# PRBonn/OverlapNet

Measured on NVIDIA H100. Metric: scan-pairs/sec (overlap+yaw) at 64x900, higher is better.
Workload: dtype f16

## Files before the change

overlapnet_b200/csrc/hopper.cuh:

```cuda
#pragma once
#include <cuda_runtime.h>
#include <stdint.h>

namespace hopper {

__device__ __forceinline__ uint32_t smem_u32(const void* p) { return (uint32_t)__cvta_generic_to_shared(p); }

__device__ __forceinline__ void mbar_init(uint64_t* bar, uint32_t count) {
  asm volatile("mbarrier.init.shared::cta.b64 [%0], %1;" :: "r"(smem_u32(bar)), "r"(count) : "memory");
}
__device__ __forceinline__ void mbar_fence_init() { asm volatile("fence.mbarrier_init.release.cluster;" ::: "memory"); }
__device__ __forceinline__ void mbar_arrive(uint64_t* bar) {
  asm volatile("{\n\t.reg .b64 st;\n\tmbarrier.arrive.shared::cta.b64 st, [%0];\n\t}\n" :: "r"(smem_u32(bar)) : "memory");
}
__device__ __forceinline__ void mbar_arrive_expect_tx(uint64_t* bar, uint32_t bytes) {
  asm volatile("{\n\t.reg .b64 st;\n\tmbarrier.arrive.expect_tx.shared::cta.b64 st, [%0], %1;\n\t}\n"
               :: "r"(smem_u32(bar)), "r"(bytes) : "memory");
}
__device__ __forceinline__ bool mbar_try_wait(uint64_t* bar, uint32_t parity) {
  uint32_t ok;
  asm volatile("{\n\t.reg .pred p;\n\tmbarrier.try_wait.parity.shared::cta.b64 p, [%1], %2;\n\tselp.u32 %0, 1, 0, p;\n\t}\n"
               : "=r"(ok) : "r"(smem_u32(bar)), "r"(parity) : "memory");
  return ok != 0;
}
__device__ __forceinline__ bool mbar_wait(uint64_t* bar, uint32_t parity, long long max_cycles) {
  if (mbar_try_wait(bar, parity)) return true;
  const long long t0 = clock64();
  while (!mbar_try_wait(bar, parity))
    if (clock64() - t0 > max_cycles) return false;
  return true;
}
constexpr long long kMbarWaitCycles = 1ll << 28;

template <int D>
struct MbarRing {
  uint64_t full[D], empty[D];
  __device__ __forceinline__ void init(uint32_t consumer_arrivals) {
    for (int s = 0; s < D; ++s) { mbar_init(&full[s], 1); mbar_init(&empty[s], consumer_arrivals); }
  }
  static __device__ __forceinline__ uint32_t slot(uint32_t i) { return i % D; }
  static __device__ __forceinline__ uint32_t parity(uint32_t i) { return (i / D) & 1; }
  __device__ __forceinline__ bool acquire(uint32_t i, uint32_t bytes) {
    if (!mbar_wait(&empty[slot(i)], parity(i) ^ 1, kMbarWaitCycles)) return false;
    mbar_arrive_expect_tx(&full[slot(i)], bytes);
    return true;
  }
  __device__ __forceinline__ bool try_acquire(uint32_t i, uint32_t bytes) {
    if (!mbar_try_wait(&empty[slot(i)], parity(i) ^ 1)) return false;
    mbar_arrive_expect_tx(&full[slot(i)], bytes);
    return true;
  }
  __device__ __forceinline__ uint64_t* bar(uint32_t i) { return &full[slot(i)]; }
  __device__ __forceinline__ bool wait(uint32_t i) { return mbar_wait(&full[slot(i)], parity(i), kMbarWaitCycles); }
  __device__ __forceinline__ void release(uint32_t i) {
    __syncwarp();
    if ((threadIdx.x & 31) == 0) mbar_arrive(&empty[slot(i)]);
  }
};

#define PIPE_WAIT(ok, code) \
  if (!(ok)) { atomicExch(err, (code)); goto done; }
#define INFLIGHT_WAIT(ok, code) \
  if (!failed && !(ok)) { atomicExch(err, (code)); failed = true; }

__device__ __forceinline__ void named_bar_sync(int id, int count) {
  asm volatile("bar.sync %0, %1;" :: "r"(id), "r"(count) : "memory");
}

__device__ __forceinline__ void bulk_g2s(void* smem_dst, const void* gmem_src, uint32_t bytes, uint64_t* bar) {
  asm volatile("cp.async.bulk.shared::cluster.global.mbarrier::complete_tx::bytes [%0], [%1], %2, [%3];"
               :: "r"(smem_u32(smem_dst)), "l"(gmem_src), "r"(bytes), "r"(smem_u32(bar)) : "memory");
}

constexpr uint32_t kNoSwizzle = 0, kSwizzle128B = 1;
__device__ __forceinline__ uint64_t desc_kmajor(uint32_t smem_addr, uint32_t lbo, uint32_t sbo, uint32_t layout) {
  return (uint64_t)((smem_addr >> 4) & 0x3FFF) | ((uint64_t)((lbo >> 4) & 0x3FFF) << 16) |
         ((uint64_t)((sbo >> 4) & 0x3FFF) << 32) | ((uint64_t)layout << 62);
}
__device__ __forceinline__ void wgmma_fence() { asm volatile("wgmma.fence.sync.aligned;" ::: "memory"); }
__device__ __forceinline__ void wgmma_commit() { asm volatile("wgmma.commit_group.sync.aligned;" ::: "memory"); }
template <int N>
__device__ __forceinline__ void wgmma_wait() { asm volatile("wgmma.wait_group.sync.aligned %0;" :: "n"(N) : "memory"); }

__device__ __forceinline__ void wgmma_m64n64k16_rs(float (&d)[32], const uint32_t (&a)[4], uint64_t b_desc) {
  asm volatile(
      "{\n\t.reg .pred p;\n\tsetp.ne.b32 p, %37, 0;\n\t"
      "wgmma.mma_async.sync.aligned.m64n64k16.f32.f16.f16 {%0, %1, %2, %3, %4, %5, %6, %7, %8, %9, %10, %11, %12, %13, %14, %15, %16, %17, %18, %19, %20, %21, %22, %23, %24, %25, %26, %27, %28, %29, %30, %31}, {%32, %33, %34, %35}, %36, p, 1, 1, 0;\n\t}\n"
      : "+f"(d[0]), "+f"(d[1]), "+f"(d[2]), "+f"(d[3]), "+f"(d[4]), "+f"(d[5]), "+f"(d[6]), "+f"(d[7]), "+f"(d[8]), "+f"(d[9]), "+f"(d[10]), "+f"(d[11]), "+f"(d[12]), "+f"(d[13]), "+f"(d[14]), "+f"(d[15]), "+f"(d[16]), "+f"(d[17]), "+f"(d[18]), "+f"(d[19]), "+f"(d[20]), "+f"(d[21]), "+f"(d[22]), "+f"(d[23]), "+f"(d[24]), "+f"(d[25]), "+f"(d[26]), "+f"(d[27]), "+f"(d[28]), "+f"(d[29]), "+f"(d[30]), "+f"(d[31])
      : "r"(a[0]), "r"(a[1]), "r"(a[2]), "r"(a[3]), "l"(b_desc), "r"(1)
      : "memory");
}

__device__ __forceinline__ void wgmma_m64n128k16_ss(float (&d)[64], uint64_t a_desc, uint64_t b_desc) {
  asm volatile(
      "{\n\t.reg .pred p;\n\tsetp.ne.b32 p, %66, 0;\n\t"
      "wgmma.mma_async.sync.aligned.m64n128k16.f32.f16.f16 {%0, %1, %2, %3, %4, %5, %6, %7, %8, %9, %10, %11, %12, %13, %14, %15, %16, %17, %18, %19, %20, %21, %22, %23, %24, %25, %26, %27, %28, %29, %30, %31, %32, %33, %34, %35, %36, %37, %38, %39, %40, %41, %42, %43, %44, %45, %46, %47, %48, %49, %50, %51, %52, %53, %54, %55, %56, %57, %58, %59, %60, %61, %62, %63}, %64, %65, p, 1, 1, 0, 0;\n\t}\n"
      : "+f"(d[0]), "+f"(d[1]), "+f"(d[2]), "+f"(d[3]), "+f"(d[4]), "+f"(d[5]), "+f"(d[6]), "+f"(d[7]), "+f"(d[8]), "+f"(d[9]), "+f"(d[10]), "+f"(d[11]), "+f"(d[12]), "+f"(d[13]), "+f"(d[14]), "+f"(d[15]), "+f"(d[16]), "+f"(d[17]), "+f"(d[18]), "+f"(d[19]), "+f"(d[20]), "+f"(d[21]), "+f"(d[22]), "+f"(d[23]), "+f"(d[24]), "+f"(d[25]), "+f"(d[26]), "+f"(d[27]), "+f"(d[28]), "+f"(d[29]), "+f"(d[30]), "+f"(d[31]), "+f"(d[32]), "+f"(d[33]), "+f"(d[34]), "+f"(d[35]), "+f"(d[36]), "+f"(d[37]), "+f"(d[38]), "+f"(d[39]), "+f"(d[40]), "+f"(d[41]), "+f"(d[42]), "+f"(d[43]), "+f"(d[44]), "+f"(d[45]), "+f"(d[46]), "+f"(d[47]), "+f"(d[48]), "+f"(d[49]), "+f"(d[50]), "+f"(d[51]), "+f"(d[52]), "+f"(d[53]), "+f"(d[54]), "+f"(d[55]), "+f"(d[56]), "+f"(d[57]), "+f"(d[58]), "+f"(d[59]), "+f"(d[60]), "+f"(d[61]), "+f"(d[62]), "+f"(d[63])
      : "l"(a_desc), "l"(b_desc), "r"(1)
      : "memory");
}

}
```

overlapnet_b200/csrc/network_tc.cu:

```cuda
#include "common.cuh"
#include "hopper.cuh"

#include <cuda_fp16.h>
#include <stddef.h>
#include <stdlib.h>

namespace ovn {

using namespace hopper;

constexpr int WF = 360;
constexpr int CF = 128;
constexpr int S15 = 15;
constexpr int NB = 24;
constexpr int PAIR_ROWS = NB * NB;
constexpr int K4_PITCH = CF;

struct TcState {
  Buffer<__half> w1p;
  Buffer<__half> w2p;
  Buffer<__half> w3p;
  Buffer<float> b2eff;
  Buffer<__half> wres[kMaxLegLayers];
  Buffer<__half> actp[2];
  Buffer<float> leg_part;
  Buffer<__half> l16;
  Buffer<__half> r16;
  Buffer<__half> o1;
  Buffer<__half> x3;
  Buffer<float> partial;
  Buffer<__half> lc;
  Buffer<__half> rc;
  Buffer<float> corr_part;
  const float* pb_key = nullptr;
  int64_t pb_rows = 0;
  Buffer<__half> pb_l16;
  Buffer<__half> pb_lc;
  Buffer<float> mu;
  bool mu_set = false;
  Buffer<float> mu_o1;
  Buffer<float> mu_x3;
  Buffer<float> b2base;
  Buffer<float> b3eff;
  bool act_set = false;
  int64_t rows_pad = 0;
};

void TcStateDelete::operator()(TcState* t) const { delete t; }

__host__ __device__ __forceinline__ int k4_pos(int r, int c) {
  const int k = c & 31;
  return (((c >> 5) ^ (r & 1)) << 5) + ((k & 7) >> 1) * 8 + (k >> 3) * 2 + (k & 1);
}

__global__ void __launch_bounds__(256)
k_gather_rows_f16(const float* __restrict__ bank, const int32_t* __restrict__ idx, int n, const float* __restrict__ mu,
                  int row_shift, __half* __restrict__ out) {
  const int64_t per = (int64_t)WF * CF / 4;
  const int64_t i = (int64_t)blockIdx.x * blockDim.x + threadIdx.x;
  if (i >= (int64_t)n * per) return;
  const int p = (int)(i / per);
  const int64_t e = i % per;
  const int64_t row = idx ? idx[p] : p;
  const int r = (int)(e / (CF / 4)), c4 = (int)(e % (CF / 4));
  int64_t rs = r + row_shift;
  if (rs >= WF) rs -= WF;
  const float4 v = __ldg(reinterpret_cast<const float4*>(bank + (row * WF + rs) * CF) + c4);
  const float4 m = __ldg(reinterpret_cast<const float4*>(mu) + c4);
  __half2 a = __floats2half2_rn(v.x - m.x, v.y - m.y), b = __floats2half2_rn(v.z - m.z, v.w - m.w);
  __half* o = out + ((int64_t)p * WF + r) * K4_PITCH;
  *reinterpret_cast<uint32_t*>(o + k4_pos(r, 4 * c4)) = *reinterpret_cast<uint32_t*>(&a);
  *reinterpret_cast<uint32_t*>(o + k4_pos(r, 4 * c4 + 2)) = *reinterpret_cast<uint32_t*>(&b);
}

__global__ void __launch_bounds__(1024)
k_channel_mean(const float* __restrict__ bank, const int32_t* __restrict__ idx, int n, float* __restrict__ mu) {
  __shared__ float part[8][CF];
  const int c = threadIdx.x & (CF - 1), g = threadIdx.x >> 7;
  float acc = 0.f;
  for (int v = 0; v < n; ++v) {
    const float* vol = bank + (int64_t)(idx ? idx[v] : v) * WF * CF;
    for (int r = g; r < WF; r += 8) acc += __ldg(vol + (int64_t)r * CF + c);
  }
  part[g][c] = acc;
  __syncthreads();
  if (g == 0) {
    float t = 0.f;
    for (int k = 0; k < 8; ++k) t += part[k][c];
    mu[c] = __half2float(__float2half_rn(t / (float)((int64_t)n * WF)));
  }
}

constexpr int K4_STEPS = 60;

__host__ __device__ __forceinline__ size_t o1_chunk_offset(int64_t m, int di, int c8) {
  const int r = (int)(m & 127);
  return ((size_t)((m >> 7) * S15 + di) * 128 + r) * 64 + (size_t)((c8 ^ (r & 7)) * 8);
}

struct LegArgs {
  const __half* A; int64_t a_pitch;
  int runs_per_img, in_img_planes, in_run_planes;
  int kh, kw, c8in;
  const __half* Bp;
  const float* bias; int n_valid;
  int64_t M;
  __half* out_planes; int64_t out_pitch; int out_run_planes;
  float* out_f32;
  int n_split; float* part;
};

constexpr int C6_LROWS = 64, C6_RROWS = 128;
constexpr int C6_LT = 6, C6_RT = 3;
constexpr int C6_L_BYTES = 2 * 16 * C6_LROWS * 16;
constexpr int C6_R_BYTES = 2 * 16 * C6_RROWS * 16;
constexpr int C6_VOL_L_BYTES = C6_LT * C6_L_BYTES;
constexpr int C6_VOL_R_BYTES = C6_RT * C6_R_BYTES;

template <int TR, int NT>
__global__ void __launch_bounds__(256)
k_pack_corr(const float* __restrict__ bank, const int32_t* __restrict__ idx, int n, __half* __restrict__ out) {
  const int64_t i = (int64_t)blockIdx.x * blockDim.x + threadIdx.x;
  const int64_t per = 16 * NT * TR;
  if (i >= (int64_t)n * per) return;
  const int p = (int)(i / per);
  int r = (int)(i % per);
  const int vrow = r % (NT * TR); r /= NT * TR;
  const int pl = r;
  const int tile = vrow / TR, row = vrow % TR;
  float v[8];
  if (vrow < WF) {
    const int64_t src = (idx ? idx[p] : p);
    const float4 a = __ldg(reinterpret_cast<const float4*>(bank + (src * WF + vrow) * CF + pl * 8));
    const float4 b = __ldg(reinterpret_cast<const float4*>(bank + (src * WF + vrow) * CF + pl * 8 + 4));
    v[0] = a.x; v[1] = a.y; v[2] = a.z; v[3] = a.w; v[4] = b.x; v[5] = b.y; v[6] = b.z; v[7] = b.w;
  } else {
#pragma unroll
    for (int e = 0; e < 8; ++e) v[e] = 0.f;
  }
  __half hi[8], lo[8];
#pragma unroll
  for (int e = 0; e < 8; ++e) {
    hi[e] = __float2half_rn(v[e]);
    lo[e] = __float2half_rn(v[e] - __half2float(hi[e]));
  }
  __half* base = out + ((size_t)p * NT + tile) * (2 * 16 * TR * 8);
  *reinterpret_cast<uint4*>(base + ((size_t)pl * TR + row) * 8) = *reinterpret_cast<const uint4*>(hi);
  *reinterpret_cast<uint4*>(base + ((size_t)(16 + pl) * TR + row) * 8) = *reinterpret_cast<const uint4*>(lo);
}

constexpr int MMA_THREADS = 128;
constexpr int MMA_ROWS = 64;

__device__ __forceinline__ void mma16816(float (&d)[4], uint32_t a0, uint32_t a1, uint32_t a2, uint32_t a3,
                                         uint32_t b0, uint32_t b1) {
  asm volatile("mma.sync.aligned.m16n8k16.row.col.f32.f16.f16.f32 {%0,%1,%2,%3}, {%4,%5,%6,%7}, {%8,%9}, {%0,%1,%2,%3};"
               : "+f"(d[0]), "+f"(d[1]), "+f"(d[2]), "+f"(d[3])
               : "r"(a0), "r"(a1), "r"(a2), "r"(a3), "r"(b0), "r"(b1));
}

__device__ __forceinline__ uint32_t ld_h2(const __half* p) { return __ldg(reinterpret_cast<const unsigned int*>(p)); }

__device__ __forceinline__ uint32_t absdiff_h2(uint32_t a, uint32_t b) {
  const __half2 d = __hsub2(*reinterpret_cast<const __half2*>(&a), *reinterpret_cast<const __half2*>(&b));
  return *reinterpret_cast<const uint32_t*>(&d) & 0x7fff7fffu;
}

__device__ __forceinline__ uint32_t pack_h2(float a, float b) {
  const __half2 h = __floats2half2_rn(a, b);
  return *reinterpret_cast<const uint32_t*>(&h);
}

constexpr int K4_WG = 3;
constexpr int K4_THREADS = K4_WG * 128 + 32;
constexpr int K4_GROUP = 5;
constexpr int K4_NGROUPS = K4_STEPS / K4_GROUP;
static_assert(S15 % K4_GROUP == 0, "a W1 group within one 32-channel chunk");
constexpr int K4_RING = 4;
constexpr int K4_BSLICE = 4096;
constexpr uint32_t K4_VOL_BYTES = WF * K4_PITCH * 2;
constexpr uint32_t K4_RWIN_BYTES = S15 * K4_PITCH * 2;

struct K4Smem {
  __half L[WF * K4_PITCH];
  __half Rw[2][S15 * K4_PITCH];
  __half B[K4_RING][K4_GROUP * K4_BSLICE / 2];
  MbarRing<K4_RING> w1;
  MbarRing<1> left;
  MbarRing<2> right;
};
static_assert(sizeof(K4Smem) <= 232448, "k_delta_conv1_wgmma shared memory");
static_assert(offsetof(K4Smem, B) % 16 == 0 && offsetof(K4Smem, Rw) % 16 == 0, "bulk-copy alignment");

struct Share { int64_t begin, end; };
__device__ __forceinline__ Share work_share(int64_t n, uint32_t part, uint32_t parts) {
  return {n * part / parts, n * (part + 1) / parts};
}

__global__ void __launch_bounds__(K4_THREADS, 1)
k_delta_conv1_wgmma(const __half* __restrict__ L16, const int32_t* __restrict__ l_idx, const __half* __restrict__ R16,
                    int r_per_pair, const __half* __restrict__ W1p, const float* __restrict__ mu_o1,
                    __half* __restrict__ o1, int n_pairs, int* __restrict__ err) {
  extern __shared__ __align__(128) uint8_t smem_raw[];
  K4Smem& S = *reinterpret_cast<K4Smem*>(smem_raw);
  const int tid = threadIdx.x, warp = tid >> 5, lane = tid & 31;
  const Share share = work_share((int64_t)n_pairs * NB, blockIdx.x, gridDim.x);
  const int u_begin = (int)share.begin, u_end = (int)share.end;
  if (tid == 0) {
    S.w1.init(K4_WG * 4);
    S.left.init(K4_WG * 4);
    S.right.init(K4_WG * 4);
    mbar_fence_init();
  }
  __syncthreads();

  if (warp == K4_WG * 4) {
    if (lane == 0) {
      uint32_t pi = 0, gi = 0, ui = 0;
      for (int u = u_begin; u < u_end; ++u, ++ui) {
        const int p = u / NB, jb = u - p * NB;
        if (u == u_begin || jb == 0) {
          PIPE_WAIT(S.left.acquire(pi, K4_VOL_BYTES), kErrDeltaLeftProducer);
          bulk_g2s(S.L, L16 + (size_t)(l_idx ? l_idx[p] : p) * WF * K4_PITCH, K4_VOL_BYTES, S.left.bar(pi));
          ++pi;
        }
        PIPE_WAIT(S.right.acquire(ui, K4_RWIN_BYTES), kErrDeltaRightProducer);
        bulk_g2s(S.Rw[S.right.slot(ui)], R16 + (r_per_pair ? (size_t)p * WF * K4_PITCH : 0) + (size_t)jb * S15 * K4_PITCH,
                 K4_RWIN_BYTES, S.right.bar(ui));
        for (int grp = 0; grp < K4_NGROUPS; ++grp, ++gi) {
          PIPE_WAIT(S.w1.acquire(gi, K4_GROUP * K4_BSLICE), kErrDeltaW1Producer);
          bulk_g2s(S.B[S.w1.slot(gi)], W1p + (size_t)grp * K4_GROUP * (K4_BSLICE / 2), K4_GROUP * K4_BSLICE, S.w1.bar(gi));
        }
      }
    }
  } else {
    const int wg = warp >> 2, wi = warp & 3, g = lane >> 2, t = lane & 3;
    int rows[2][2];
#pragma unroll
    for (int tt = 0; tt < 2; ++tt) {
      const int r = (wg + 3 * tt) * 64 + wi * 16 + g;
      rows[tt][0] = r;
      rows[tt][1] = r + 8;
    }
    const uint32_t b_base = smem_u32(S.B[0]);
    uint32_t pi = 0, gi = 0, ui = 0;
    for (int u = u_begin; u < u_end; ++u, ++ui) {
      const int p = u / NB, jb = u - p * NB;
      if (u == u_begin || jb == 0) { PIPE_WAIT(S.left.wait(pi), kErrDeltaLeftConsumer); ++pi; }
      const uint32_t wb = S.right.slot(ui);
      PIPE_WAIT(S.right.wait(ui), kErrDeltaRightConsumer);
      float acc[2][32];
#pragma unroll
      for (int j = 0; j < 8; ++j) {
        const float m0 = __half2float(__float2half_rn(-__ldg(mu_o1 + j * 8 + 2 * t)));
        const float m1 = __half2float(__float2half_rn(-__ldg(mu_o1 + j * 8 + 2 * t + 1)));
#pragma unroll
        for (int tt = 0; tt < 2; ++tt) {
          acc[tt][4 * j + 0] = m0; acc[tt][4 * j + 1] = m1;
          acc[tt][4 * j + 2] = m0; acc[tt][4 * j + 3] = m1;
        }
      }
      uint32_t Lr[2][2][4];
#pragma unroll 1
      for (int grp = 0; grp < K4_NGROUPS; ++grp, ++gi) {
        const int cc = grp / 3, dj0 = (grp - 3 * cc) * K4_GROUP;
        if (dj0 == 0) {
#pragma unroll
          for (int tt = 0; tt < 2; ++tt)
#pragma unroll
            for (int h = 0; h < 2; ++h) {
              const int r = rows[tt][h] < WF ? rows[tt][h] : WF - 1;
              const uint4 v = *reinterpret_cast<const uint4*>(S.L + r * K4_PITCH + ((cc ^ (r & 1)) << 5) + 8 * t);
              Lr[tt][h][0] = v.x; Lr[tt][h][1] = v.y; Lr[tt][h][2] = v.z; Lr[tt][h][3] = v.w;
            }
        }
        const uint32_t s = S.w1.slot(gi);
        const uint64_t bdesc = desc_kmajor(b_base + s * (K4_GROUP * K4_BSLICE), 1024, 128, kNoSwizzle);
        const int par = (jb + dj0) & 1;
        const __half* rw = S.Rw[wb] + dj0 * K4_PITCH + 8 * t;
        const __half* rp[2] = {rw + ((cc ^ par) << 5), rw + ((cc ^ par ^ 1) << 5)};
        uint4 rv = *reinterpret_cast<const uint4*>(rp[0]);
        PIPE_WAIT(S.w1.wait(gi), kErrDeltaW1Consumer);
#pragma unroll
        for (int sl = 0; sl < K4_GROUP; ++sl) {
          uint32_t A[2][2][4];
#pragma unroll
          for (int tt = 0; tt < 2; ++tt) {
            A[tt][0][0] = absdiff_h2(Lr[tt][0][0], rv.x);
            A[tt][0][1] = absdiff_h2(Lr[tt][1][0], rv.x);
            A[tt][0][2] = absdiff_h2(Lr[tt][0][1], rv.y);
            A[tt][0][3] = absdiff_h2(Lr[tt][1][1], rv.y);
            A[tt][1][0] = absdiff_h2(Lr[tt][0][2], rv.z);
            A[tt][1][1] = absdiff_h2(Lr[tt][1][2], rv.z);
            A[tt][1][2] = absdiff_h2(Lr[tt][0][3], rv.w);
            A[tt][1][3] = absdiff_h2(Lr[tt][1][3], rv.w);
          }
          wgmma_fence();
#pragma unroll
          for (int kk = 0; kk < 2; ++kk)
#pragma unroll
            for (int tt = 0; tt < 2; ++tt)
              wgmma_m64n64k16_rs(acc[tt], A[tt][kk], bdesc + ((sl * K4_BSLICE + kk * 2048) >> 4));
          wgmma_commit();
          if (sl + 1 < K4_GROUP) rv = *reinterpret_cast<const uint4*>(rp[(sl + 1) & 1] + (sl + 1) * K4_PITCH);
          wgmma_wait<0>();
        }
        S.w1.release(gi);
      }
      S.right.release(ui);
      if (jb == NB - 1 || u == u_end - 1) S.left.release(pi - 1);
      const int64_t mrow = (int64_t)p * PAIR_ROWS + jb * NB;
#pragma unroll
      for (int tt = 0; tt < 2; ++tt)
#pragma unroll
        for (int h = 0; h < 2; ++h) {
          const int i = rows[tt][h];
          if (i >= WF) continue;
          const int ibk = i / S15, di = i - ibk * S15;
#pragma unroll
          for (int j = 0; j < 8; ++j)
            *reinterpret_cast<uint32_t*>(o1 + o1_chunk_offset(mrow + ibk, di, j) + 2 * t) =
                pack_h2(acc[tt][4 * j + 2 * h], acc[tt][4 * j + 2 * h + 1]);
        }
    }
  }
done:
  return;
}

constexpr int TC_WG = 2;
constexpr int TC_THREADS = TC_WG * 128 + 32;
constexpr int TC_ROWS = TC_WG * 128;
constexpr uint32_t C2_TILE = 128 * 64 * 2;
constexpr int C2_RING = 3;

struct C2Smem {
  __half A[C2_RING][TC_WG][C2_TILE / 2];
  __half B[C2_RING][2][C2_TILE / 2];
  MbarRing<C2_RING> ring;
};
constexpr size_t C2_SMEM = sizeof(C2Smem) + 1024;
static_assert(C2_SMEM <= 232448, "k_conv2_wgmma shared memory");
static_assert(offsetof(C2Smem, B) % 1024 == 0 && C2_TILE % 1024 == 0, "SWIZZLE_128B tiles on 1024-byte boundaries");

__global__ void __launch_bounds__(TC_THREADS, 1)
k_conv2_wgmma(const __half* __restrict__ o1, const __half* __restrict__ W2s, const float* __restrict__ bias2,
              const float* __restrict__ mu_x3, __half* __restrict__ x3, int64_t out_pitch, int64_t M, int fault,
              int* __restrict__ err) {
  if (fault) {
    if (threadIdx.x == 0 && blockIdx.x == 0) atomicExch(err, kErrInjectedFault);
    return;
  }
  extern __shared__ __align__(128) uint8_t smem_raw[];
  C2Smem& S = *reinterpret_cast<C2Smem*>(smem_raw + ((1024 - (smem_u32(smem_raw) & 1023)) & 1023));
  const int tid = threadIdx.x, warp = tid >> 5, lane = tid & 31;
  const Share tiles = work_share((M + TC_ROWS - 1) / TC_ROWS, blockIdx.x, gridDim.x);
  if (tid == 0) {
    S.ring.init(TC_WG * 4);
    mbar_fence_init();
  }
  __syncthreads();

  if (warp == TC_WG * 4) {
    if (lane == 0) {
      uint32_t gi = 0;
      for (int64_t tile = tiles.begin; tile < tiles.end; ++tile)
        for (int di = 0; di < S15; ++di, ++gi) {
          const uint32_t s = S.ring.slot(gi);
          PIPE_WAIT(S.ring.acquire(gi, 4 * C2_TILE), kErrConv2Producer);
          for (int h = 0; h < TC_WG; ++h)
            bulk_g2s(S.A[s][h], o1 + ((size_t)(tile * TC_WG + h) * S15 + di) * (C2_TILE / 2), C2_TILE, S.ring.bar(gi));
          bulk_g2s(S.B[s], W2s + (size_t)di * C2_TILE, 2 * C2_TILE, S.ring.bar(gi));
        }
    }
  } else {
    const int wg = warp >> 2, wi = warp & 3, g = lane >> 2, t = lane & 3;
    uint32_t gi = 0;
    bool failed = false;
    for (int64_t tile = tiles.begin; tile < tiles.end; ++tile) {
      float acc[2][64];
#pragma unroll
      for (int sub = 0; sub < 2; ++sub)
#pragma unroll
        for (int e = 0; e < 64; ++e) acc[sub][e] = 0.f;
#pragma unroll 1
      for (int di = 0; di < S15; ++di, ++gi) {
        const uint32_t s = S.ring.slot(gi);
        INFLIGHT_WAIT(S.ring.wait(gi), kErrConv2Consumer);
        const uint32_t a_base = smem_u32(S.A[s][wg]), b_base = smem_u32(S.B[s][0]);
        wgmma_fence();
#pragma unroll
        for (int kk = 0; kk < 4; ++kk)
#pragma unroll
          for (int part = 0; part < 2; ++part) {
            const uint64_t bd = desc_kmajor(b_base + part * C2_TILE + kk * 32, 16, 1024, kSwizzle128B);
#pragma unroll
            for (int sub = 0; sub < 2; ++sub)
              wgmma_m64n128k16_ss(acc[sub], desc_kmajor(a_base + sub * (C2_TILE / 2) + kk * 32, 16, 1024, kSwizzle128B), bd);
          }
        wgmma_commit();
        wgmma_wait<1>();
        if (di > 0) S.ring.release(gi - 1);
      }
      wgmma_wait<0>();
      if (failed) goto done;
      S.ring.release(gi - 1);
#pragma unroll
      for (int sub = 0; sub < 2; ++sub)
#pragma unroll
        for (int h = 0; h < 2; ++h) {
          const int64_t m = tile * TC_ROWS + wg * 128 + sub * 64 + wi * 16 + g + 8 * h;
          if (m >= M) continue;
#pragma unroll
          for (int j = 0; j < 16; ++j) {
            const int n = j * 8 + 2 * t;
            const float a = fmaxf(acc[sub][4 * j + 2 * h] + __ldg(bias2 + n), 0.f) - __ldg(mu_x3 + n);
            const float b = fmaxf(acc[sub][4 * j + 2 * h + 1] + __ldg(bias2 + n + 1), 0.f) - __ldg(mu_x3 + n + 1);
            *reinterpret_cast<uint32_t*>(x3 + ((size_t)j * out_pitch + m) * 8 + 2 * t) = pack_h2(a, b);
          }
        }
    }
  }
done:
  return;
}

constexpr int C3_AROWS = TC_ROWS + 2 * NB + 2;
constexpr uint32_t C3_PLANE = C3_AROWS * 16;
constexpr uint32_t C3_SLAB = 4 * 128 * 16;
constexpr int C3_GROUP = 2;
constexpr int C3_NSTAGES = 36 / C3_GROUP;
constexpr int C3_RING = 4;

struct C3Smem {
  __half A[2][16 * C3_PLANE / 2];
  __half B[C3_RING][C3_GROUP * C3_SLAB / 2];
  MbarRing<C3_RING> w3;
  MbarRing<2> x3;
};
static_assert(sizeof(C3Smem) <= 232448, "k_conv3_wgmma shared memory");
static_assert(offsetof(C3Smem, B) % 16 == 0 && C3_PLANE % 16 == 0, "bulk-copy alignment");

__global__ void __launch_bounds__(TC_THREADS, 1)
k_conv3_wgmma(const __half* __restrict__ X3, int64_t a_pitch, const __half* __restrict__ W3p, const float* __restrict__ bias,
              int64_t M, const float* __restrict__ wd, float* __restrict__ partial, int* __restrict__ err) {
  extern __shared__ __align__(128) uint8_t smem_raw[];
  C3Smem& S = *reinterpret_cast<C3Smem*>(smem_raw);
  const int tid = threadIdx.x, warp = tid >> 5, lane = tid & 31;
  const Share tiles = work_share(2 * ((M + TC_ROWS - 1) / TC_ROWS), blockIdx.x, gridDim.x);
  if (tid == 0) {
    S.w3.init(TC_WG * 4);
    S.x3.init(TC_WG * 4);
    mbar_fence_init();
  }
  __syncthreads();

  if (warp == TC_WG * 4) {
    if (lane == 0) {
      const uint32_t nt = (uint32_t)(tiles.end - tiles.begin);
      uint32_t ai = 0, gi = 0;
      for (uint32_t ti = 0; ti < nt; ++ti) {
        const int nh = (int)((tiles.begin + ti) & 1);
        for (int st = 0; st < C3_NSTAGES; ++st, ++gi) {
          while (ai < nt && ai <= ti + 1) {
            if (ai > ti) {
              if (!S.x3.try_acquire(ai, 16 * C3_PLANE)) break;
            } else {
              PIPE_WAIT(S.x3.acquire(ai, 16 * C3_PLANE), kErrConv3X3Producer);
            }
            const int64_t r0 = ((tiles.begin + ai) >> 1) * TC_ROWS;
            for (int pl = 0; pl < 16; ++pl)
              bulk_g2s(S.A[S.x3.slot(ai)] + pl * (C3_PLANE / 2), X3 + ((size_t)pl * a_pitch + r0) * 8, C3_PLANE, S.x3.bar(ai));
            ++ai;
          }
          PIPE_WAIT(S.w3.acquire(gi, C3_GROUP * C3_SLAB), kErrConv3W3Producer);
          bulk_g2s(S.B[S.w3.slot(gi)], W3p + ((size_t)nh * 36 + st * C3_GROUP) * (C3_SLAB / 2), C3_GROUP * C3_SLAB,
                   S.w3.bar(gi));
        }
      }
    }
  } else {
    const int wg = warp >> 2, wi = warp & 3, g = lane >> 2, t = lane & 3;
    const uint32_t b_base = smem_u32(S.B[0]);
    uint32_t gi = 0;
    bool failed = false;
    for (int64_t tile = tiles.begin; tile < tiles.end; ++tile) {
      const uint32_t ti = (uint32_t)(tile - tiles.begin);
      const int nh = (int)(tile & 1);
      const int64_t r0 = (tile >> 1) * TC_ROWS;
      PIPE_WAIT(S.x3.wait(ti), kErrConv3X3Consumer);
      const uint32_t a_rows = smem_u32(S.A[S.x3.slot(ti)]) + wg * 128 * 16;
      float acc[2][64];
#pragma unroll
      for (int sub = 0; sub < 2; ++sub)
#pragma unroll
        for (int e = 0; e < 64; ++e) acc[sub][e] = 0.f;
#pragma unroll 1
      for (int st = 0; st < C3_NSTAGES; ++st, ++gi) {
        const uint32_t s = S.w3.slot(gi);
        INFLIGHT_WAIT(S.w3.wait(gi), kErrConv3W3Consumer);
        wgmma_fence();
#pragma unroll
        for (int sl = 0; sl < C3_GROUP; ++sl) {
          const int slab = st * C3_GROUP + sl, tap = slab >> 2, c32 = slab & 3;
          const uint32_t a_tap = a_rows + ((tap / 3) * NB + tap % 3) * 16;
          const uint32_t slab_addr = b_base + s * (C3_GROUP * C3_SLAB) + sl * C3_SLAB;
#pragma unroll
          for (int kk = 0; kk < 2; ++kk) {
            const int c16 = c32 * 2 + kk;
            const uint64_t bd = desc_kmajor(slab_addr + kk * 4096, 2048, 128, kNoSwizzle);
#pragma unroll
            for (int sub = 0; sub < 2; ++sub)
              wgmma_m64n128k16_ss(acc[sub], desc_kmajor(a_tap + 2 * c16 * C3_PLANE + sub * 64 * 16, C3_PLANE, 128, kNoSwizzle), bd);
          }
        }
        wgmma_commit();
        wgmma_wait<1>();
        if (st > 0) S.w3.release(gi - 1);
      }
      wgmma_wait<0>();
      if (failed) goto done;
      S.w3.release(gi - 1);
      S.x3.release(ti);
#pragma unroll
      for (int sub = 0; sub < 2; ++sub)
#pragma unroll
        for (int h = 0; h < 2; ++h) {
          const int64_t r = r0 + wg * 128 + sub * 64 + wi * 16 + g + 8 * h;
          const int rem = (int)(r % PAIR_ROWS);
          const int yy = rem / NB, xx = rem - yy * NB;
          const bool valid = (r < M) && (yy < NB - 2) && (xx < NB - 2);
          const float* wrow = wd + (size_t)(valid ? (xx * (NB - 2) + yy) : 0) * 256 + nh * 128;
          float sum = 0.f;
#pragma unroll
          for (int j = 0; j < 16; ++j) {
            const int n = j * 8 + 2 * t;
            sum = fmaf(fmaxf(acc[sub][4 * j + 2 * h] + __ldg(bias + nh * 128 + n), 0.f), __ldg(wrow + n), sum);
            sum = fmaf(fmaxf(acc[sub][4 * j + 2 * h + 1] + __ldg(bias + nh * 128 + n + 1), 0.f), __ldg(wrow + n + 1), sum);
          }
          sum += __shfl_xor_sync(0xffffffffu, sum, 1);
          sum += __shfl_xor_sync(0xffffffffu, sum, 2);
          if (t == 0 && r < M) partial[r * 2 + nh] = valid ? sum : 0.f;
        }
    }
  }
done:
  return;
}

constexpr int C6_PARTS = C6_LT * C6_RT;
constexpr int C6_WG = 2;
constexpr int C6_THREADS = C6_WG * 128 + 32;
constexpr int C6_RING = 3;
constexpr int C6_GPITCH = 132;

struct C6Smem {
  __half R[C6_R_BYTES / 2];
  __half L[C6_RING][C6_L_BYTES / 2];
  float G[C6_WG][C6_LROWS * C6_GPITCH];
  MbarRing<C6_RING> left;
  MbarRing<1> right;
};
static_assert(sizeof(C6Smem) <= 232448, "k_corr_wgmma shared memory");
static_assert(offsetof(C6Smem, L) % 16 == 0, "bulk-copy alignment");

__global__ void __launch_bounds__(C6_THREADS, 1)
k_corr_wgmma(const __half* __restrict__ Lc, const int32_t* __restrict__ l_idx, const __half* __restrict__ Rc,
             int r_per_pair, int n_pairs, float* __restrict__ corr_part, int* __restrict__ err) {
  extern __shared__ __align__(128) uint8_t smem_raw[];
  C6Smem& S = *reinterpret_cast<C6Smem*>(smem_raw);
  const int tid = threadIdx.x, warp = tid >> 5, lane = tid & 31;
  const int q = blockIdx.x % C6_RT;
  const Share share = work_share((int64_t)n_pairs * C6_LT, blockIdx.x / C6_RT, gridDim.x / C6_RT);
  const int u_begin = (int)share.begin, u_end = (int)share.end;
  if (tid == 0) {
    S.left.init(4);
    S.right.init(C6_WG * 4);
    mbar_fence_init();
  }
  __syncthreads();

  if (warp == C6_WG * 4) {
    if (lane == 0) {
      uint32_t ri = 0, ui = 0;
      int key = -1;
      for (int u = u_begin; u < u_end; ++u, ++ui) {
        const int p = u / C6_LT, a = u - p * C6_LT;
        if ((r_per_pair ? p : 0) != key) {
          key = r_per_pair ? p : 0;
          PIPE_WAIT(S.right.acquire(ri, C6_R_BYTES), kErrCorrRightProducer);
          bulk_g2s(S.R, Rc + ((size_t)key * C6_RT + q) * (C6_R_BYTES / 2), C6_R_BYTES, S.right.bar(ri));
          ++ri;
        }
        PIPE_WAIT(S.left.acquire(ui, C6_L_BYTES), kErrCorrLeftProducer);
        bulk_g2s(S.L[S.left.slot(ui)], Lc + ((size_t)(l_idx ? l_idx[p] : p) * C6_LT + a) * (C6_L_BYTES / 2), C6_L_BYTES,
                 S.left.bar(ui));
      }
    }
  } else {
    const int wg = warp >> 2, wi = warp & 3, g = lane >> 2, t = lane & 3, tw = tid & 127;
    float* Gw = S.G[wg];
    const uint32_t r_base = smem_u32(S.R);
    uint32_t ri = 0, ui = 0;
    int key = -1;
    bool failed = false;
    for (int u = u_begin; u < u_end; ++u, ++ui) {
      const int p = u / C6_LT, a = u - p * C6_LT;
      if ((r_per_pair ? p : 0) != key) {
        if (key >= 0) S.right.release(ri - 1);
// ... 803 lines not shown
```

Before: 148,600.

## Widen producer to a warpgroup with setmaxnreg and overlap wgmma k-halves

The producer grows from a single warp to a full warpgroup so setmaxnreg can be used: producer warps drop to 32 registers and consumer warpgroups rise to 160. The inner loop now builds the absdiff A fragments per k-half, commits each half as its own wgmma group, and waits with wait_group 1. This lets the next half's fragment math overlap the in-flight MMA instead of fully draining after every slice. The cost is 96 extra idle threads per block, and reusing the A array while an earlier wgmma may still be reading its register operands carries a hazard risk.

```diff
diff --git a/overlapnet_b200/csrc/hopper.cuh b/overlapnet_b200/csrc/hopper.cuh
--- a/overlapnet_b200/csrc/hopper.cuh
+++ b/overlapnet_b200/csrc/hopper.cuh
@@ -67,6 +67,11 @@
   asm volatile("bar.sync %0, %1;" :: "r"(id), "r"(count) : "memory");
 }
 
+template <uint32_t N>
+__device__ __forceinline__ void setmaxnreg_dec() { asm volatile("setmaxnreg.dec.sync.aligned.u32 %0;" :: "n"(N)); }
+template <uint32_t N>
+__device__ __forceinline__ void setmaxnreg_inc() { asm volatile("setmaxnreg.inc.sync.aligned.u32 %0;" :: "n"(N)); }
+
 __device__ __forceinline__ void bulk_g2s(void* smem_dst, const void* gmem_src, uint32_t bytes, uint64_t* bar) {
   asm volatile("cp.async.bulk.shared::cluster.global.mbarrier::complete_tx::bytes [%0], [%1], %2, [%3];"
                :: "r"(smem_u32(smem_dst)), "l"(gmem_src), "r"(bytes), "r"(smem_u32(bar)) : "memory");
diff --git a/overlapnet_b200/csrc/network_tc.cu b/overlapnet_b200/csrc/network_tc.cu
--- a/overlapnet_b200/csrc/network_tc.cu
+++ b/overlapnet_b200/csrc/network_tc.cu
@@ -172,7 +172,8 @@
 }
 
 constexpr int K4_WG = 3;
-constexpr int K4_THREADS = K4_WG * 128 + 32;
+constexpr int K4_THREADS = (K4_WG + 1) * 128;
+constexpr uint32_t K4_REG_PRODUCER = 32, K4_REG_CONSUMER = 160;
 constexpr int K4_GROUP = 5;
 constexpr int K4_NGROUPS = K4_STEPS / K4_GROUP;
 static_assert(S15 % K4_GROUP == 0, "a W1 group within one 32-channel chunk");
@@ -214,8 +215,9 @@
   }
   __syncthreads();
 
-  if (warp == K4_WG * 4) {
-    if (lane == 0) {
+  if (warp >= K4_WG * 4) {
+    setmaxnreg_dec<K4_REG_PRODUCER>();
+    if (warp == K4_WG * 4 && lane == 0) {
       uint32_t pi = 0, gi = 0, ui = 0;
       for (int u = u_begin; u < u_end; ++u, ++ui) {
         const int p = u / NB, jb = u - p * NB;
@@ -234,6 +236,7 @@
       }
     }
   } else {
+    setmaxnreg_inc<K4_REG_CONSUMER>();
     const int wg = warp >> 2, wi = warp & 3, g = lane >> 2, t = lane & 3;
     int rows[2][2];
 #pragma unroll
@@ -281,30 +284,28 @@
         const __half* rp[2] = {rw + ((cc ^ par) << 5), rw + ((cc ^ par ^ 1) << 5)};
         uint4 rv = *reinterpret_cast<const uint4*>(rp[0]);
         PIPE_WAIT(S.w1.wait(gi), kErrDeltaW1Consumer);
-#pragma unroll
-        for (int sl = 0; sl < K4_GROUP; ++sl) {
-          uint32_t A[2][2][4];
-#pragma unroll
-          for (int tt = 0; tt < 2; ++tt) {
-            A[tt][0][0] = absdiff_h2(Lr[tt][0][0], rv.x);
-            A[tt][0][1] = absdiff_h2(Lr[tt][1][0], rv.x);
-            A[tt][0][2] = absdiff_h2(Lr[tt][0][1], rv.y);
-            A[tt][0][3] = absdiff_h2(Lr[tt][1][1], rv.y);
-            A[tt][1][0] = absdiff_h2(Lr[tt][0][2], rv.z);
-            A[tt][1][1] = absdiff_h2(Lr[tt][1][2], rv.z);
-            A[tt][1][2] = absdiff_h2(Lr[tt][0][3], rv.w);
-            A[tt][1][3] = absdiff_h2(Lr[tt][1][3], rv.w);
-          }
-          wgmma_fence();
-#pragma unroll
-          for (int kk = 0; kk < 2; ++kk)
+        uint32_t A[2][2][4];
+#pragma unroll
+        for (int sl = 0; sl < K4_GROUP; ++sl)
+#pragma unroll
+          for (int kk = 0; kk < 2; ++kk) {
+            const uint32_t r0 = kk ? rv.z : rv.x, r1 = kk ? rv.w : rv.y;
+#pragma unroll
+            for (int tt = 0; tt < 2; ++tt) {
+              A[tt][kk][0] = absdiff_h2(Lr[tt][0][2 * kk], r0);
+              A[tt][kk][1] = absdiff_h2(Lr[tt][1][2 * kk], r0);
+              A[tt][kk][2] = absdiff_h2(Lr[tt][0][2 * kk + 1], r1);
+              A[tt][kk][3] = absdiff_h2(Lr[tt][1][2 * kk + 1], r1);
+            }
+            wgmma_fence();
 #pragma unroll
             for (int tt = 0; tt < 2; ++tt)
               wgmma_m64n64k16_rs(acc[tt], A[tt][kk], bdesc + ((sl * K4_BSLICE + kk * 2048) >> 4));
-          wgmma_commit();
-          if (sl + 1 < K4_GROUP) rv = *reinterpret_cast<const uint4*>(rp[(sl + 1) & 1] + (sl + 1) * K4_PITCH);
-          wgmma_wait<0>();
-        }
+            wgmma_commit();
+            if (kk == 1 && sl + 1 < K4_GROUP) rv = *reinterpret_cast<const uint4*>(rp[(sl + 1) & 1] + (sl + 1) * K4_PITCH);
+            wgmma_wait<1>();
+          }
+        wgmma_wait<0>();
         S.w1.release(gi);
       }
       S.right.release(ui);
```

Result: faster. 161,800 (median of 6 runs) (+8.8%).
